# nimiq/snark-setup-operator

Measured on NVIDIA B200. Metric: phase1_contribute_points_per_s, higher is better.
Workload: dtype u32 limbs (Montgomery, integer pipe)

## Files before the change

### snark-setup-operator_b200/csrc/coop.cuh

```cuda
#pragma once
#include "ext.cuh"
#ifdef SSO_HOST_EMUL
#include <atomic>
#include <thread>
#include <functional>
#endif

namespace sso {

#ifndef SSO_HOST_EMUL
template <int DEG> struct Coop {
  static_assert(DEG == 2 || DEG == 3, "two or three lanes per element");
  static constexpr uint32_t GROUPS_PER_WARP = 32 / DEG;
  __device__ __forceinline__ static uint32_t lane() { return threadIdx.x & 31u; }
  __device__ __forceinline__ static uint32_t role() { return DEG == 2 ? (threadIdx.x & 1u) : (threadIdx.x & 31u) % 3u; }
  __device__ __forceinline__ static uint32_t base() { return lane() - role(); }
  __device__ __forceinline__ static uint32_t mask() { return ((1u << DEG) - 1u) << base(); }
  __device__ __forceinline__ static bool lane_active() { return lane() < GROUPS_PER_WARP * DEG; }
  __device__ __forceinline__ static uint32_t group_in_block() { return (threadIdx.x >> 5) * GROUPS_PER_WARP + lane() / DEG; }
  template <int N> __device__ __forceinline__ static void rot(uint32_t* out, const uint32_t* in, uint32_t k) {
    uint32_t r = role() + k;
    if (r >= DEG) r -= DEG;
    const uint32_t src = base() + r, m = mask();
#pragma unroll
    for (int i = 0; i < N; i++) out[i] = __shfl_sync(m, in[i], src);
  }
  __device__ __forceinline__ static uint32_t get(uint32_t v, uint32_t from) { return __shfl_sync(mask(), v, base() + from); }
  __device__ __forceinline__ static bool all(bool c) { return __all_sync(mask(), c) != 0; }
};
#else
struct CoopEmuState {
  std::atomic<int> count{0};
  std::atomic<int> sense{0};
  const uint32_t* slot[3] = {nullptr, nullptr, nullptr};
  uint32_t flag[3] = {0, 0, 0};
  int lanes = 1;
};
inline CoopEmuState& coop_emu() { static CoopEmuState s; return s; }
static thread_local int g_coop_role = 0;
static thread_local int g_coop_sense = 0;
inline void coop_emu_barrier() {
  CoopEmuState& s = coop_emu();
  g_coop_sense ^= 1;
  if (s.count.fetch_add(1) + 1 == s.lanes) { s.count.store(0); s.sense.store(g_coop_sense); }
  else while (s.sense.load() != g_coop_sense) std::this_thread::yield();
}
inline void coop_emu_run(int deg, const std::function<void(int)>& fn) {
  CoopEmuState& s = coop_emu();
  s.lanes = deg; s.count.store(0); s.sense.store(0);
  std::vector<std::thread> th;
  for (int r = 0; r < deg; r++) th.emplace_back([&, r] { g_coop_role = r; g_coop_sense = 0; fn(r); });
  for (auto& t : th) t.join();
}
template <int DEG> struct Coop {
  static uint32_t role() { return (uint32_t)g_coop_role; }
  template <int N> static void rot(uint32_t* out, const uint32_t* in, uint32_t k) {
    CoopEmuState& s = coop_emu();
    uint32_t tmp[N];
    s.slot[g_coop_role] = in;
    coop_emu_barrier();
    const uint32_t* src = s.slot[(g_coop_role + k) % DEG];
    for (int i = 0; i < N; i++) tmp[i] = src[i];
    coop_emu_barrier();
    for (int i = 0; i < N; i++) out[i] = tmp[i];
  }
  static uint32_t get(uint32_t v, uint32_t from) {
    CoopEmuState& s = coop_emu();
    s.flag[g_coop_role] = v;
    coop_emu_barrier();
    uint32_t r = s.flag[from];
    coop_emu_barrier();
    return r;
  }
  static bool all(bool c) {
    CoopEmuState& s = coop_emu();
    s.flag[g_coop_role] = c ? 1u : 0u;
    coop_emu_barrier();
    bool r = true;
    for (int i = 0; i < DEG; i++) r = r && s.flag[i] != 0;
    coop_emu_barrier();
    return r;
  }
};
#endif

template <int N> __device__ __forceinline__ void sel_words(uint32_t* out, bool c, const uint32_t* a, const uint32_t* b) {
#pragma unroll
  for (int i = 0; i < N; i++) out[i] = c ? a[i] : b[i];
}

template <class B_, int K, bool NEG> struct CFp2 {
  using B = B_;
  using Base = B_;
  using NR = SmallNR<B_, K, NEG>;
  using CO = Coop<2>;
  static constexpr int DEG = 2;
  static constexpr int COOP = 2;
  static constexpr bool LAZY_OK = !NEG && B_::SPARE_BITS >= 15;
  static constexpr bool SQR_CHEAPER = true;
  static constexpr int L = B::L;
  static constexpr int NBYTES = 2 * B::NBYTES;
  static constexpr int WORDS = 2 * B::L;
  using T = typename B::T;

  __device__ __forceinline__ static T pick(bool c, const T& a, const T& b) { T r; sel_words<L>(r.v, c, a.v, b.v); return r; }
  __device__ __forceinline__ static T other(const T& a) { T o; CO::template rot<L>(o.v, a.v, 1); return o; }

  __device__ __forceinline__ static T zero() { return B::zero(); }
  __device__ __forceinline__ static T one() { return pick(CO::role() == 0, B::one(), B::zero()); }
  __device__ __forceinline__ static bool is_zero(const T& a) { return CO::all(B::is_zero(a)); }
  __device__ __forceinline__ static bool eq(const T& a, const T& b) { return CO::all(B::eq(a, b)); }
  __device__ __forceinline__ static T add(const T& a, const T& b) { return B::add(a, b); }
  __device__ __forceinline__ static T sub(const T& a, const T& b) { return B::sub(a, b); }
  __device__ __forceinline__ static T dbl(const T& a) { return B::dbl(a); }
  __device__ __forceinline__ static T neg(const T& a) { return B::neg(a); }
  template <int M> __device__ __forceinline__ static T mul_small(const T& a) { return B::template mul_small<M>(a); }
  __device__ __forceinline__ static T add_lazy(const T& a, const T& b) { return B::add_lazy(a, b); }
  __device__ __forceinline__ static T sub_lazy(const T& a, const T& b) { return B::sub_lazy(a, b); }
  __device__ __forceinline__ static T mad_small_lazy(const T& c, uint32_t k, const T& x) { return B::mad_small_lazy(c, k, x); }

  __device__ __noinline__ static T mul_val(T a, T b) {
    const bool hi = CO::role() != 0;
    T ob = other(b);
    T x = NEG ? pick(hi, B::neg_lazy(b), b) : b;
    T kb = B::mad_small_lazy(B::zero(), hi ? (uint32_t)K : 1u, x);
    T ps = B::mul(a, kb);
    T pc = B::mul(a, ob);
    T recv = other(pick(hi, ps, pc));
    return B::add(pick(hi, pc, ps), recv);
  }
  __device__ __noinline__ static T sqr_val(T a) {
    static_assert((K & 1) == 1, "odd non-residue");
    constexpr int H = (NEG ? K - 1 : K + 1) / 2;
    const bool hi = CO::role() != 0;
    T o = other(a);
    T X = B::add_lazy(a, pick(hi, a, o));
    T Y = B::mad_small_lazy(pick(hi, o, a), hi ? 0u : (uint32_t)K, NEG ? B::neg_lazy(o) : o);
    T P = B::mul(X, Y);
    T w = other(P);
    return B::reduce_small(B::mad_small_lazy(P, hi ? 0u : (uint32_t)H, NEG ? w : B::neg_lazy(w)));
  }
  __device__ __forceinline__ static T mul(const T& a, const T& b) { return mul_val(a, b); }
  __device__ __forceinline__ static T sqr(const T& a) { return sqr_val(a); }
  __device__ __forceinline__ static T mul_base(const T& a, const typename B::T& k) { return B::mul(a, k); }
  __device__ __forceinline__ static T conj(const T& a) { return pick(CO::role() != 0, B::neg(a), a); }
  __device__ __noinline__ static T inv(const T& a) {
    const bool hi = CO::role() != 0;
    T sq = B::sqr(a);
    T osq = other(sq);
    T n = B::sub(pick(hi, osq, sq), NR::mul(pick(hi, sq, osq)));
    T ni = B::inv(n);
    T r = B::mul(a, ni);
    return pick(hi, B::neg(r), r);
  }
  __device__ __forceinline__ static bool from_bytes(const uint8_t* src, bool with_flags, uint32_t& flags, T& out) {
    const uint32_t r = CO::role();
    uint32_t f = 0;
    bool ok = B::from_bytes(src + r * B::NBYTES, with_flags && r == 1, f, out);
    flags = CO::get(f, 1);
    return CO::all(ok);
  }
  __device__ __forceinline__ static T load(const uint32_t* p, size_t stride) { return B::load(p + (size_t)CO::role() * L * stride, stride); }
  __device__ __forceinline__ static void store(uint32_t* p, size_t stride, const T& a) { B::store(p + (size_t)CO::role() * L * stride, stride, a); }
  __device__ __forceinline__ static T from_const(const uint32_t* c) { return B::from_const(c + CO::role() * L); }
};

template <class B_, int K, bool NEG> struct CFp3 {
  using B = B_;
  using Base = B_;
  using NR = SmallNR<B_, K, NEG>;
  using CO = Coop<3>;
  static constexpr int DEG = 3;
  static constexpr int COOP = 3;
  static constexpr bool LAZY_OK = B_::SPARE_BITS >= 15;
  static constexpr bool SQR_CHEAPER = false;
  static constexpr int L = B::L;
  static constexpr int NBYTES = 3 * B::NBYTES;
  static constexpr int WORDS = 3 * B::L;
  using T = typename B::T;

  __device__ __forceinline__ static T pick(bool c, const T& a, const T& b) { T r; sel_words<L>(r.v, c, a.v, b.v); return r; }
  __device__ __forceinline__ static T from(const T& a, uint32_t k) { T o; CO::template rot<L>(o.v, a.v, k); return o; }

  __device__ __forceinline__ static T zero() { return B::zero(); }
  __device__ __forceinline__ static T one() { return pick(CO::role() == 0, B::one(), B::zero()); }
  __device__ __forceinline__ static bool is_zero(const T& a) { return CO::all(B::is_zero(a)); }
  __device__ __forceinline__ static bool eq(const T& a, const T& b) { return CO::all(B::eq(a, b)); }
  __device__ __forceinline__ static T add(const T& a, const T& b) { return B::add(a, b); }
  __device__ __forceinline__ static T sub(const T& a, const T& b) { return B::sub(a, b); }
  __device__ __forceinline__ static T dbl(const T& a) { return B::dbl(a); }
  __device__ __forceinline__ static T neg(const T& a) { return B::neg(a); }
  template <int M> __device__ __forceinline__ static T mul_small(const T& a) { return B::template mul_small<M>(a); }
  __device__ __forceinline__ static T add_lazy(const T& a, const T& b) { return B::add_lazy(a, b); }
  __device__ __forceinline__ static T sub_lazy(const T& a, const T& b) { return B::sub_lazy(a, b); }
  __device__ __forceinline__ static T mad_small_lazy(const T& c, uint32_t k, const T& x) { return B::mad_small_lazy(c, k, x); }

  __device__ __noinline__ static T mul_val(T a, T b) {
    static_assert(!NEG, "positive non-residue");
    const uint32_t r = CO::role();
    T v = B::mul(a, b);
    T s = B::mul(B::add_lazy(a, from(a, 1)), B::add_lazy(b, from(b, 1)));
    T u = B::sub(s, v);
    T r1 = from(pick(r == 1, u, v), 1);
    T r2 = from(pick(r == 0, u, v), 2);
    T d = B::sub(pick(r == 0, r1, pick(r == 1, r2, u)), pick(r == 0, r2, pick(r == 1, v, r1)));
    return B::reduce_small(B::mad_small_lazy(pick(r == 0, v, d), r == 2 ? 1u : (uint32_t)K, pick(r == 0, d, pick(r == 1, r1, r2))));
  }
  __device__ __forceinline__ static T mul(const T& a, const T& b) { return mul_val(a, b); }
  __device__ __forceinline__ static T sqr(const T& a) { return mul_val(a, a); }
  __device__ __forceinline__ static T mul_base(const T& a, const typename B::T& k) { return B::mul(a, k); }
  __device__ __noinline__ static T inv(const T& a) {
    const uint32_t r = CO::role();
    T an = from(a, 1), ap = from(a, 2);
    T sq = B::sqr(pick(r == 0, a, pick(r == 1, an, ap)));
    T pr = B::mul(pick(r == 1, ap, an), pick(r == 0, ap, a));
    T nrs = NR::mul(pick(r == 0, pr, sq));
    T t = B::sub(pick(r == 1, nrs, sq), pick(r == 0, nrs, pr));
    T m = B::mul(pick(r == 0, a, pick(r == 1, an, ap)), t);
    T mn = from(m, 1), mp = from(m, 2);
    T cand = B::add(m, NR::mul(B::add(mn, mp)));
    T n = from(cand, r == 0 ? 0u : 3u - r);
    return B::mul(t, B::inv(n));
  }
  __device__ __forceinline__ static T frob_w(const T& a, const uint32_t* w1, const uint32_t* w2) {
    const uint32_t r = CO::role();
    T m = B::mul(a, pick(r == 1, B::from_const(w1), B::from_const(w2)));
    return pick(r == 0, a, m);
  }
  __device__ __forceinline__ static T mul_u2(const T& a) {
    const uint32_t r = CO::role();
    T n = from(a, 1);
    return pick(r == 2, n, NR::mul(n));
  }
  __device__ __forceinline__ static bool from_bytes(const uint8_t* src, bool with_flags, uint32_t& flags, T& out) {
    const uint32_t r = CO::role();
    uint32_t f = 0;
    bool ok = B::from_bytes(src + r * B::NBYTES, with_flags && r == 2, f, out);
    flags = CO::get(f, 2);
    return CO::all(ok);
  }
  __device__ __forceinline__ static T load(const uint32_t* p, size_t stride) { return B::load(p + (size_t)CO::role() * L * stride, stride); }
  __device__ __forceinline__ static void store(uint32_t* p, size_t stride, const T& a) { B::store(p + (size_t)CO::role() * L * stride, stride, a); }
  __device__ __forceinline__ static T from_const(const uint32_t* c) { return B::from_const(c + CO::role() * L); }
};

}
```

### snark-setup-operator_b200/csrc/fp.cuh

```cuda
#pragma once
#include <cstdint>
#include "constants.cuh"

#ifndef SSO_INLINE_MUL_MAX_L
#define SSO_INLINE_MUL_MAX_L 8
#endif

#ifndef SSO_SQR_EC_MAX_L
#define SSO_SQR_EC_MAX_L 12
#endif
#ifndef SSO_LAZY_TRADE_ALL
#define SSO_LAZY_TRADE_ALL 0
#endif

namespace sso {

#ifndef SSO_HOST_EMUL
__device__ __forceinline__ uint32_t add_cc(uint32_t a, uint32_t b) { uint32_t r; asm volatile("add.cc.u32 %0, %1, %2;" : "=r"(r) : "r"(a), "r"(b)); return r; }
__device__ __forceinline__ uint32_t addc_cc(uint32_t a, uint32_t b) { uint32_t r; asm volatile("addc.cc.u32 %0, %1, %2;" : "=r"(r) : "r"(a), "r"(b)); return r; }
__device__ __forceinline__ uint32_t addc(uint32_t a, uint32_t b) { uint32_t r; asm volatile("addc.u32 %0, %1, %2;" : "=r"(r) : "r"(a), "r"(b)); return r; }
__device__ __forceinline__ uint32_t sub_cc(uint32_t a, uint32_t b) { uint32_t r; asm volatile("sub.cc.u32 %0, %1, %2;" : "=r"(r) : "r"(a), "r"(b)); return r; }
__device__ __forceinline__ uint32_t subc_cc(uint32_t a, uint32_t b) { uint32_t r; asm volatile("subc.cc.u32 %0, %1, %2;" : "=r"(r) : "r"(a), "r"(b)); return r; }
__device__ __forceinline__ uint32_t subc(uint32_t a, uint32_t b) { uint32_t r; asm volatile("subc.u32 %0, %1, %2;" : "=r"(r) : "r"(a), "r"(b)); return r; }
__device__ __forceinline__ uint32_t mul_lo(uint32_t a, uint32_t b) { uint32_t r; asm volatile("mul.lo.u32 %0, %1, %2;" : "=r"(r) : "r"(a), "r"(b)); return r; }
__device__ __forceinline__ uint32_t mul_hi(uint32_t a, uint32_t b) { uint32_t r; asm volatile("mul.hi.u32 %0, %1, %2;" : "=r"(r) : "r"(a), "r"(b)); return r; }
__device__ __forceinline__ uint64_t mul_wide(uint32_t a, uint32_t b) { uint64_t r; asm volatile("mul.wide.u32 %0, %1, %2;" : "=l"(r) : "r"(a), "r"(b)); return r; }
__device__ __forceinline__ uint32_t mad_lo_cc(uint32_t a, uint32_t b, uint32_t c) { uint32_t r; asm volatile("mad.lo.cc.u32 %0, %1, %2, %3;" : "=r"(r) : "r"(a), "r"(b), "r"(c)); return r; }
__device__ __forceinline__ uint32_t madc_lo_cc(uint32_t a, uint32_t b, uint32_t c) { uint32_t r; asm volatile("madc.lo.cc.u32 %0, %1, %2, %3;" : "=r"(r) : "r"(a), "r"(b), "r"(c)); return r; }
__device__ __forceinline__ uint32_t madc_hi_cc(uint32_t a, uint32_t b, uint32_t c) { uint32_t r; asm volatile("madc.hi.cc.u32 %0, %1, %2, %3;" : "=r"(r) : "r"(a), "r"(b), "r"(c)); return r; }
__device__ __forceinline__ uint32_t madc_hi(uint32_t a, uint32_t b, uint32_t c) { uint32_t r; asm volatile("madc.hi.u32 %0, %1, %2, %3;" : "=r"(r) : "r"(a), "r"(b), "r"(c)); return r; }
__device__ __forceinline__ uint32_t shl1_from(uint32_t lo, uint32_t hi) { return __funnelshift_l(lo, hi, 1); }
#else
static thread_local uint32_t g_cf = 0;
static inline uint32_t emu_add(uint32_t a, uint32_t b, uint32_t cin, bool setc) { uint64_t s = (uint64_t)a + b + cin; if (setc) g_cf = (uint32_t)(s >> 32); return (uint32_t)s; }
static inline uint32_t emu_sub(uint32_t a, uint32_t b, uint32_t bin, bool setc) { uint64_t s = (uint64_t)a - b - bin; if (setc) g_cf = (uint32_t)((s >> 32) & 1); return (uint32_t)s; }
static inline uint32_t add_cc(uint32_t a, uint32_t b) { return emu_add(a, b, 0, true); }
static inline uint32_t addc_cc(uint32_t a, uint32_t b) { return emu_add(a, b, g_cf, true); }
static inline uint32_t addc(uint32_t a, uint32_t b) { return emu_add(a, b, g_cf, false); }
static inline uint32_t sub_cc(uint32_t a, uint32_t b) { return emu_sub(a, b, 0, true); }
static inline uint32_t subc_cc(uint32_t a, uint32_t b) { return emu_sub(a, b, g_cf, true); }
static inline uint32_t subc(uint32_t a, uint32_t b) { return emu_sub(a, b, g_cf, false); }
static inline uint32_t mul_lo(uint32_t a, uint32_t b) { return (uint32_t)((uint64_t)a * b); }
static inline uint32_t mul_hi(uint32_t a, uint32_t b) { return (uint32_t)(((uint64_t)a * b) >> 32); }
static inline uint64_t mul_wide(uint32_t a, uint32_t b) { return (uint64_t)a * b; }
static inline uint32_t mad_lo_cc(uint32_t a, uint32_t b, uint32_t c) { return emu_add(mul_lo(a, b), c, 0, true); }
static inline uint32_t madc_lo_cc(uint32_t a, uint32_t b, uint32_t c) { return emu_add(mul_lo(a, b), c, g_cf, true); }
static inline uint32_t madc_hi_cc(uint32_t a, uint32_t b, uint32_t c) { return emu_add(mul_hi(a, b), c, g_cf, true); }
static inline uint32_t madc_hi(uint32_t a, uint32_t b, uint32_t c) { return emu_add(mul_hi(a, b), c, g_cf, false); }
static inline uint32_t shl1_from(uint32_t lo, uint32_t hi) { return (hi << 1) | (lo >> 31); }
static inline int __popc(uint32_t x) { return __builtin_popcount(x); }
static inline int __clz(uint32_t x) { return x ? __builtin_clz(x) : 32; }
#endif

template <int N> struct big { uint32_t v[N]; };

template <int N> __device__ __forceinline__ bool limbs_is_zero(const uint32_t* a) {
  uint32_t o = 0;
#pragma unroll
  for (int i = 0; i < N; i++) o |= a[i];
  return o == 0;
}
template <int N> __device__ __forceinline__ bool limbs_eq(const uint32_t* a, const uint32_t* b) {
  uint32_t o = 0;
#pragma unroll
  for (int i = 0; i < N; i++) o |= a[i] ^ b[i];
  return o == 0;
}
template <int N> __device__ __forceinline__ bool limbs_gt(const uint32_t* a, const uint32_t* b) {
  sub_cc(b[0], a[0]);
#pragma unroll
  for (int i = 1; i < N; i++) subc_cc(b[i], a[i]);
  return subc(0, 0) != 0;
}
template <int N> __device__ __forceinline__ uint32_t limbs_add(uint32_t* r, const uint32_t* a, const uint32_t* b) {
  r[0] = add_cc(a[0], b[0]);
#pragma unroll
  for (int i = 1; i < N; i++) r[i] = addc_cc(a[i], b[i]);
  return addc(0, 0);
}
template <int N> __device__ __forceinline__ uint32_t limbs_sub(uint32_t* r, const uint32_t* a, const uint32_t* b) {
  r[0] = sub_cc(a[0], b[0]);
#pragma unroll
  for (int i = 1; i < N; i++) r[i] = subc_cc(a[i], b[i]);
  return subc(0, 0);
}

template <int n> __device__ __forceinline__ void mul_n(uint32_t* acc, const uint32_t* a, uint32_t bi) {
#pragma unroll
  for (int j = 0; j < n; j += 2) {
    uint64_t t = mul_wide(a[j], bi);
    acc[j] = (uint32_t)t;
    acc[j + 1] = (uint32_t)(t >> 32);
  }
}
template <int n> __device__ __forceinline__ void cmad_n(uint32_t* acc, const uint32_t* a, uint32_t bi) {
  acc[0] = mad_lo_cc(a[0], bi, acc[0]);
  acc[1] = madc_hi_cc(a[0], bi, acc[1]);
#pragma unroll
  for (int j = 2; j < n; j += 2) {
    acc[j] = madc_lo_cc(a[j], bi, acc[j]);
    acc[j + 1] = madc_hi_cc(a[j], bi, acc[j + 1]);
  }
}
template <int n> __device__ __forceinline__ void madc_n_rshift(uint32_t* acc, const uint32_t* a, uint32_t bi) {
#pragma unroll
  for (int j = 0; j < n - 2; j += 2) {
    acc[j] = madc_lo_cc(a[j], bi, acc[j + 2]);
    acc[j + 1] = madc_hi_cc(a[j], bi, acc[j + 3]);
  }
  acc[n - 2] = madc_lo_cc(a[n - 2], bi, 0);
  acc[n - 1] = madc_hi(a[n - 2], bi, 0);
}

template <class P> __device__ __forceinline__ void load_modulus(uint32_t* mod) {
#pragma unroll
  for (int i = 0; i < P::L; i++) mod[i] = P::p()[i];
}

template <class P> __device__ __forceinline__ void mad_n_redc(uint32_t* E, uint32_t* O, const uint32_t* a, uint32_t bi, bool first,
                                                              const uint32_t* MOD) {
  constexpr int n = P::L;
  if (first) {
    mul_n<n>(O, a + 1, bi);
    mul_n<n>(E, a, bi);
  } else {
    E[0] = add_cc(E[0], O[1]);
    madc_n_rshift<n>(O, a + 1, bi);
    cmad_n<n>(E, a, bi);
    O[n - 1] = addc(O[n - 1], 0);
  }
  uint32_t mi = E[0] * P::inv_rt();
  cmad_n<n>(O, MOD + 1, mi);
  cmad_n<n>(E, MOD, mi);
  O[n - 1] = addc(O[n - 1], 0);
}

template <class P> __device__ __forceinline__ void mont_mul(uint32_t* r, const uint32_t* a, const uint32_t* b) {
  constexpr int n = P::L;
  uint32_t even[n], odd[n], mod[n];
  load_modulus<P>(mod);
#pragma unroll
  for (int i = 0; i < n; i += 2) {
    mad_n_redc<P>(even, odd, a, b[i], i == 0, mod);
    mad_n_redc<P>(odd, even, a, b[i + 1], false, mod);
  }
  even[0] = add_cc(even[0], odd[1]);
#pragma unroll
  for (int k = 1; k < n - 1; k++) even[k] = addc_cc(even[k], odd[k + 1]);
  even[n - 1] = addc(even[n - 1], 0);
  uint32_t t[n];
  uint32_t borrow = limbs_sub<n>(t, even, mod);
#pragma unroll
  for (int k = 0; k < n; k++) r[k] = borrow ? even[k] : t[k];
}

template <int n, int i, int j0> __device__ __forceinline__ void sqr_row(uint32_t* acc, const uint32_t* a) {
  if constexpr (j0 < n) {
    acc[i + j0] = mad_lo_cc(a[i], a[j0], acc[i + j0]);
    acc[i + j0 + 1] = madc_hi_cc(a[i], a[j0], acc[i + j0 + 1]);
    constexpr int last = j0 + 2 * ((n - 1 - j0) / 2);
#pragma unroll
    for (int j = j0 + 2; j < n; j += 2) {
      acc[i + j] = madc_lo_cc(a[i], a[j], acc[i + j]);
      acc[i + j + 1] = madc_hi_cc(a[i], a[j], acc[i + j + 1]);
    }
    acc[i + last + 2] = addc(acc[i + last + 2], 0);
  }
}
template <int n, int i> __device__ __forceinline__ void sqr_rows(uint32_t* ev, uint32_t* od, const uint32_t* a) {
  if constexpr (i < n - 1) {
    sqr_row<n, i, i + 1>(od, a);
    sqr_row<n, i, i + 2>(ev, a);
    sqr_rows<n, i + 1>(ev, od, a);
  }
}
template <int n> __device__ __forceinline__ void sqr_wide(uint32_t* w, const uint32_t* a) {
  uint32_t ev[2 * n], od[2 * n];
#pragma unroll
  for (int k = 0; k < 2 * n; k++) { ev[k] = 0; od[k] = 0; }
  sqr_rows<n, 0>(ev, od, a);
  ev[1] = add_cc(ev[1], od[1]);
#pragma unroll
  for (int k = 2; k < 2 * n - 1; k++) ev[k] = addc_cc(ev[k], od[k]);
  ev[2 * n - 1] = addc(ev[2 * n - 1], od[2 * n - 1]);
  w[0] = mad_lo_cc(a[0], a[0], 0);
  w[1] = madc_hi_cc(a[0], a[0], ev[1] << 1);
#pragma unroll
  for (int i = 1; i < n; i++) {
    w[2 * i] = madc_lo_cc(a[i], a[i], shl1_from(ev[2 * i - 1], ev[2 * i]));
    w[2 * i + 1] = i == n - 1 ? madc_hi(a[i], a[i], shl1_from(ev[2 * i], ev[2 * i + 1]))
                              : madc_hi_cc(a[i], a[i], shl1_from(ev[2 * i], ev[2 * i + 1]));
  }
}
template <class P> __device__ __forceinline__ void redc_step(uint32_t* E, uint32_t* O, bool first, const uint32_t* MOD) {
  constexpr int n = P::L;
  if (first) {
    uint32_t mi = E[0] * P::inv_rt();
    mul_n<n>(O, MOD + 1, mi);
    cmad_n<n>(E, MOD, mi);
    O[n - 1] = addc(O[n - 1], 0);
  } else {
    uint32_t mi = (E[0] + O[1]) * P::inv_rt();
    E[0] = add_cc(E[0], O[1]);
    madc_n_rshift<n>(O, MOD + 1, mi);
    cmad_n<n>(E, MOD, mi);
    O[n - 1] = addc(O[n - 1], 0);
  }
}
template <class P> __device__ __forceinline__ void mont_sqr(uint32_t* r, const uint32_t* a) {
  constexpr int n = P::L;
  uint32_t w[2 * n], odd[n], mod[n];
  sqr_wide<n>(w, a);
  load_modulus<P>(mod);
  uint32_t* even = w;
#pragma unroll
  for (int i = 0; i < n; i += 2) {
    redc_step<P>(even, odd, i == 0, mod);
    redc_step<P>(odd, even, false, mod);
  }
  even[0] = add_cc(even[0], odd[1]);
#pragma unroll
  for (int k = 1; k < n - 1; k++) even[k] = addc_cc(even[k], odd[k + 1]);
  even[n - 1] = addc(even[n - 1], 0);
  limbs_add<n>(even, even, w + n);
  uint32_t t[n];
  uint32_t borrow = limbs_sub<n>(t, even, mod);
#pragma unroll
  for (int k = 0; k < n; k++) r[k] = borrow ? even[k] : t[k];
}

template <class P_> struct Fp {
  using P = P_;
  static constexpr int L = P::L;
  static constexpr int DEG = 1;
  static constexpr int COOP = 0;
  static constexpr int NBYTES = P::NBYTES;
  static constexpr int WORDS = L;
  struct T { uint32_t v[L]; };
  using Base = Fp<P_>;

  __device__ __forceinline__ static T zero() { T r;
#pragma unroll
    for (int i = 0; i < L; i++) r.v[i] = 0;
    return r; }
  __device__ __forceinline__ static T one() { T r;
#pragma unroll
    for (int i = 0; i < L; i++) r.v[i] = P::r1()[i];
    return r; }
  __device__ __forceinline__ static bool is_zero(const T& a) { return limbs_is_zero<L>(a.v); }
  __device__ __forceinline__ static bool eq(const T& a, const T& b) { return limbs_eq<L>(a.v, b.v); }

  __device__ __forceinline__ static T add(const T& a, const T& b) {
    T s, t, r;
    limbs_add<L>(s.v, a.v, b.v);
    uint32_t borrow = limbs_sub<L>(t.v, s.v, P::p());
#pragma unroll
    for (int i = 0; i < L; i++) r.v[i] = borrow ? s.v[i] : t.v[i];
    return r;
  }
  __device__ __forceinline__ static T dbl(const T& a) { return add(a, a); }
  __device__ __forceinline__ static T sub(const T& a, const T& b) {
    T d, t, r;
    uint32_t borrow = limbs_sub<L>(d.v, a.v, b.v);
    limbs_add<L>(t.v, d.v, P::p());
#pragma unroll
    for (int i = 0; i < L; i++) r.v[i] = borrow ? t.v[i] : d.v[i];
    return r;
  }
  __device__ __forceinline__ static T neg(const T& a) {
    T t;
    limbs_sub<L>(t.v, P::p(), a.v);
    bool z = is_zero(a);
#pragma unroll
    for (int i = 0; i < L; i++) t.v[i] = z ? 0u : t.v[i];
    return t;
  }
  static constexpr int SPARE_BITS = 32 * L - P::BITS;
  static constexpr bool LAZY_OK = SPARE_BITS >= 7;
  static constexpr bool SQR_CHEAPER = L <= SSO_SQR_EC_MAX_L && !SSO_LAZY_TRADE_ALL;
  __device__ __forceinline__ static T add_lazy(const T& a, const T& b) { T r; limbs_add<L>(r.v, a.v, b.v); return r; }
  __device__ __forceinline__ static T neg_lazy(const T& a) { T r; limbs_sub<L>(r.v, P::p(), a.v); return r; }
  __device__ __forceinline__ static T sub_lazy(const T& a, const T& b) {
    T n, r;
    limbs_sub<L>(n.v, P::p(), b.v);
    limbs_add<L>(r.v, a.v, n.v);
    return r;
  }
  __device__ __forceinline__ static T mad_small_lazy(const T& c, uint32_t k, const T& x) {
    uint32_t ev[L], od[L];
    mul_n<L>(ev, x.v, k);
    mul_n<L>(od, x.v + 1, k);
    T r;
    r.v[0] = add_cc(c.v[0], ev[0]);
#pragma unroll
    for (int i = 1; i < L - 1; i++) r.v[i] = addc_cc(c.v[i], ev[i]);
    r.v[L - 1] = addc(c.v[L - 1], ev[L - 1]);
    r.v[1] = add_cc(r.v[1], od[0]);
#pragma unroll
    for (int i = 2; i < L - 1; i++) r.v[i] = addc_cc(r.v[i], od[i - 1]);
    r.v[L - 1] = addc(r.v[L - 1], od[L - 2]);
    return r;
  }
  __device__ __forceinline__ static T reduce_small(const T& y) {
    static_assert(SPARE_BITS >= 7 && SPARE_BITS <= 15, "top limb of p must hold at least 17 bits, and 16 p < R");
    uint32_t q = y.v[L - 1] / (P::p()[L - 1] + 1u);
    uint32_t ev[L], od[L], mod[L];
    load_modulus<P>(mod);
    mul_n<L>(ev, mod, q);
    mul_n<L>(od, mod + 1, q);
    T d;
    d.v[0] = sub_cc(y.v[0], ev[0]);
#pragma unroll
    for (int i = 1; i < L - 1; i++) d.v[i] = subc_cc(y.v[i], ev[i]);
    d.v[L - 1] = subc(y.v[L - 1], ev[L - 1]);
    d.v[1] = sub_cc(d.v[1], od[0]);
#pragma unroll
    for (int i = 2; i < L - 1; i++) d.v[i] = subc_cc(d.v[i], od[i - 1]);
    d.v[L - 1] = subc(d.v[L - 1], od[L - 2]);
    T t, r;
    uint32_t borrow = limbs_sub<L>(t.v, d.v, mod);
#pragma unroll
    for (int i = 0; i < L; i++) r.v[i] = borrow ? d.v[i] : t.v[i];
    return r;
  }

  __device__ __noinline__ static T mul_outlined(T a, T b) { T r; mont_mul<P>(r.v, a.v, b.v); return r; }
  __device__ __forceinline__ static T mul(const T& a, const T& b) {
    if constexpr (L > SSO_INLINE_MUL_MAX_L) { return mul_outlined(a, b); } else { T r; mont_mul<P>(r.v, a.v, b.v); return r; }
  }
#ifndef SSO_SQR_EC_MAX_L
#define SSO_SQR_EC_MAX_L 12
#endif
  __device__ __noinline__ static T sqr_outlined(T a) { T r; mont_sqr<P>(r.v, a.v); return r; }
  __device__ __forceinline__ static T sqr_dedicated(const T& a) {
    if constexpr (L > SSO_INLINE_MUL_MAX_L) { return sqr_outlined(a); } else { T r; mont_sqr<P>(r.v, a.v); return r; }
  }
  __device__ __forceinline__ static T sqr(const T& a) {
    if constexpr (L <= SSO_SQR_EC_MAX_L) return sqr_dedicated(a); else return mul(a, a);
  }
  __device__ __forceinline__ static T mul_inl(const T& a, const T& b) { T r; mont_mul<P>(r.v, a.v, b.v); return r; }
  template <int K> __device__ __forceinline__ static T mul_small(const T& a) {
    static_assert(K >= 0 && K < 64, "small constant");
    T acc = zero();
    T base = a;
    bool started = false;
#pragma unroll
    for (int bit = 0; bit < 6; bit++) {
      if ((K >> bit) & 1) { acc = started ? add(acc, base) : base; started = true; }
      if ((K >> (bit + 1)) != 0) base = dbl(base);
    }
    return acc;
  }

  __device__ __forceinline__ static T to_mont(const T& a) { T r2;
#pragma unroll
    for (int i = 0; i < L; i++) r2.v[i] = P::r2()[i];
    return mul(a, r2); }
  __device__ __forceinline__ static T from_mont(const T& a) { T o = zero(); o.v[0] = 1; return mul(a, o); }

  __device__ __noinline__ static T pow_const(const T& a, const uint32_t* e) {
    T r = one();
    bool started = false;
    for (int i = L * 32 - 1; i >= 0; i--) {
      if (started) r = sqr_dedicated(r);
      if ((e[i >> 5] >> (i & 31)) & 1) { r = started ? mul(r, a) : a; started = true; }
    }
    return r;
  }
  __device__ __forceinline__ static T inv_fermat(const T& a) { return pow_const(a, P::pm2()); }

  __device__ __noinline__ static T inv(const T& a) {
    if (is_zero(a)) return a;
    uint32_t u[L], v[L], x1[L], x2[L], t[L];
#pragma unroll
    for (int i = 0; i < L; i++) { u[i] = a.v[i]; v[i] = P::p()[i]; x1[i] = i == 0 ? 1u : 0u; x2[i] = 0u; }
    auto halve_mod = [&](uint32_t* x) {
      if (x[0] & 1u) limbs_add<L>(x, x, P::p());
#pragma unroll
      for (int i = 0; i < L - 1; i++) x[i] = (x[i] >> 1) | (x[i + 1] << 31);
      x[L - 1] >>= 1;
    };
    auto shr1 = [&](uint32_t* x) {
#pragma unroll
      for (int i = 0; i < L - 1; i++) x[i] = (x[i] >> 1) | (x[i + 1] << 31);
      x[L - 1] >>= 1;
    };
    auto is_one = [&](const uint32_t* x) {
      uint32_t o = x[0] ^ 1u;
#pragma unroll
      for (int i = 1; i < L; i++) o |= x[i];
      return o == 0;
    };
    while (!is_one(u) && !is_one(v)) {
      while ((u[0] & 1u) == 0) { shr1(u); halve_mod(x1); }
      while ((v[0] & 1u) == 0) { shr1(v); halve_mod(x2); }
      if (limbs_sub<L>(t, u, v) == 0) {
#pragma unroll
        for (int i = 0; i < L; i++) u[i] = t[i];
        if (limbs_sub<L>(x1, x1, x2) != 0) limbs_add<L>(x1, x1, P::p());
      } else {
        limbs_sub<L>(v, v, u);
        if (limbs_sub<L>(x2, x2, x1) != 0) limbs_add<L>(x2, x2, P::p());
      }
    }
    T r;
    bool use1 = is_one(u);
#pragma unroll
    for (int i = 0; i < L; i++) r.v[i] = use1 ? x1[i] : x2[i];
    T r2;
#pragma unroll
    for (int i = 0; i < L; i++) r2.v[i] = P::r2()[i];
    return mul(mul(r, r2), r2);
  }

  __device__ __forceinline__ static bool is_neg_canonical(const T& canon) { return limbs_gt<L>(canon.v, P::half()); }
  __device__ __forceinline__ static int sign_canonical(const T& canon) {
    if (is_zero(canon)) return 0;
    return is_neg_canonical(canon) ? 1 : -1;
  }
  __device__ __forceinline__ static bool lex_is_neg(const T& a) { return is_neg_canonical(from_mont(a)); }

  __device__ __noinline__ static bool sqrt(const T& a, T& out) {
    if (is_zero(a)) { out = a; return true; }
    if (P::P_IS_3_MOD_4) {
      T w = pow_const(a, P::tm1h());
      T x = mul(a, w);
      out = x;
      return eq(sqr(x), a);
    }
    T w = pow_const(a, P::tm1h());
    T x = mul(a, w);
    T b = mul(x, w);
    T z;
#pragma unroll
    for (int i = 0; i < L; i++) z.v[i] = P::tsz()[i];
    int m = P::TWO_ADICITY;
    T o = one();
    while (!eq(b, o)) {
      int k = 0;
      T b2 = b;
      while (!eq(b2, o)) { b2 = sqr(b2); k++; if (k >= m) return false; }
      T wz = z;
      for (int j = 0; j < m - k - 1; j++) wz = sqr(wz);
      z = sqr(wz);
      b = mul(b, z);
      x = mul(x, wz);
      m = k;
    }
    out = x;
    return true;
  }

  __device__ __forceinline__ static bool from_bytes(const uint8_t* src, bool with_flags, uint32_t& flags, T& out) {
    T c = zero();
#pragma unroll
    for (int i = 0; i < NBYTES; i++) {
      uint32_t byte = src[i];
      if (i == NBYTES - 1) {
        flags = with_flags ? (byte & 0xC0u) : 0u;
        if (with_flags) byte &= 0x3Fu;
      }
      c.v[i >> 2] |= byte << ((i & 3) * 8);
    }
    T t;
    uint32_t borrow = limbs_sub<L>(t.v, c.v, P::p());
    out = to_mont(c);
    return borrow != 0;
  }
  __device__ __forceinline__ static void to_bytes(uint8_t* dst, const T& a, uint32_t flags) {
    T c = from_mont(a);
#pragma unroll
    for (int i = 0; i < NBYTES; i++) {
      uint32_t byte = (c.v[i >> 2] >> ((i & 3) * 8)) & 0xFFu;
      if (i == NBYTES - 1) byte |= flags;
      dst[i] = (uint8_t)byte;
    }
  }
  __device__ __forceinline__ static T load(const uint32_t* p, size_t stride) { T r;
#pragma unroll
    for (int i = 0; i < L; i++) r.v[i] = p[i * stride];
    return r; }
  __device__ __forceinline__ static void store(uint32_t* p, size_t stride, const T& a) {
#pragma unroll
    for (int i = 0; i < L; i++) p[i * stride] = a.v[i];
  }
  __device__ __forceinline__ static T from_const(const uint32_t* c) { T r;
#pragma unroll
    for (int i = 0; i < L; i++) r.v[i] = c[i];
    return r; }
};

}
```

Before: 9.697 million.

## Fuse cooperative extension multiply into sum of wide products with single reduction

The cooperative Fp2 multiply now has each lane compute two double-width products (its own limb times the partner's, plus the other limb times a scaled partner value), add them unreduced, and run one Montgomery reduction. This replaces two full Montgomery multiplies, an extra shuffle exchange and a final modular add. The squaring path's reduction is factored out into a reusable redc_wide, and a new schoolbook mul_wide is added. The lazy sum of two wide products must stay within the bounds the reduction can handle, and the wider intermediates raise register pressure.

```diff
diff --git a/snark-setup-operator_b200/csrc/coop.cuh b/snark-setup-operator_b200/csrc/coop.cuh
--- a/snark-setup-operator_b200/csrc/coop.cuh
+++ b/snark-setup-operator_b200/csrc/coop.cuh
@@ -121,13 +121,16 @@
 
   __device__ __noinline__ static T mul_val(T a, T b) {
     const bool hi = CO::role() != 0;
-    T ob = other(b);
-    T x = NEG ? pick(hi, B::neg_lazy(b), b) : b;
-    T kb = B::mad_small_lazy(B::zero(), hi ? (uint32_t)K : 1u, x);
-    T ps = B::mul(a, kb);
-    T pc = B::mul(a, ob);
-    T recv = other(pick(hi, ps, pc));
-    return B::add(pick(hi, pc, ps), recv);
+    T oa = other(a), ob = other(b);
+    T x = NEG ? pick(hi, b, B::neg_lazy(ob)) : pick(hi, b, ob);
+    T y = B::mad_small_lazy(B::zero(), hi ? 1u : (uint32_t)K, x);
+    uint32_t w[2 * L], w2[2 * L];
+    mul_wide<L>(w, a.v, pick(hi, ob, b).v);
+    mul_wide<L>(w2, oa.v, y.v);
+    limbs_add<2 * L>(w, w, w2);
+    T r;
+    redc_wide<typename B::P>(r.v, w);
+    return r;
   }
   __device__ __noinline__ static T sqr_val(T a) {
     static_assert((K & 1) == 1, "odd non-residue");
diff --git a/snark-setup-operator_b200/csrc/fp.cuh b/snark-setup-operator_b200/csrc/fp.cuh
--- a/snark-setup-operator_b200/csrc/fp.cuh
+++ b/snark-setup-operator_b200/csrc/fp.cuh
@@ -207,10 +207,9 @@
     O[n - 1] = addc(O[n - 1], 0);
   }
 }
-template <class P> __device__ __forceinline__ void mont_sqr(uint32_t* r, const uint32_t* a) {
+template <class P> __device__ __forceinline__ void redc_wide(uint32_t* r, uint32_t* w) {
   constexpr int n = P::L;
-  uint32_t w[2 * n], odd[n], mod[n];
-  sqr_wide<n>(w, a);
+  uint32_t odd[n], mod[n];
   load_modulus<P>(mod);
   uint32_t* even = w;
 #pragma unroll
@@ -227,6 +226,34 @@
   uint32_t borrow = limbs_sub<n>(t, even, mod);
 #pragma unroll
   for (int k = 0; k < n; k++) r[k] = borrow ? even[k] : t[k];
+}
+template <class P> __device__ __forceinline__ void mont_sqr(uint32_t* r, const uint32_t* a) {
+  uint32_t w[2 * P::L];
+  sqr_wide<P::L>(w, a);
+  redc_wide<P>(r, w);
+}
+
+template <int n> __device__ __forceinline__ void mad_row(uint32_t* acc_o, uint32_t* acc_e, const uint32_t* a, uint32_t bi) {
+  cmad_n<n - 2>(acc_o, a + 1, bi);
+  acc_o[n - 2] = madc_lo_cc(a[n - 1], bi, 0);
+  acc_o[n - 1] = madc_hi(a[n - 1], bi, 0);
+  cmad_n<n>(acc_e, a, bi);
+  acc_o[n - 1] = addc(acc_o[n - 1], 0);
+}
+template <int n> __device__ __forceinline__ void mul_wide(uint32_t* w, const uint32_t* a, const uint32_t* b) {
+  uint32_t od[2 * n - 2];
+  mul_n<n>(w, a, b[0]);
+  mul_n<n>(od, a + 1, b[0]);
+  mad_row<n>(w + 2, od, a, b[1]);
+#pragma unroll
+  for (int i = 2; i < n - 1; i += 2) {
+    mad_row<n>(od + i, w + i, a, b[i]);
+    mad_row<n>(w + i + 2, od + i, a, b[i + 1]);
+  }
+  w[1] = add_cc(w[1], od[0]);
+#pragma unroll
+  for (int k = 2; k < 2 * n - 1; k++) w[k] = addc_cc(w[k], od[k - 1]);
+  w[2 * n - 1] = addc(w[2 * n - 1], 0);
 }
 
 template <class P_> struct Fp {
```

After: 9.696 million, median of 6. No clear change (-0.0%).
